# Seasandwpy/viso

Measured on AMD Instinct MI355X. Metric: stereo frames/sec at 1242x375 grey, 1/2/4/8 GPUs; pose RMSE vs reference, higher is better.
Workload: dtype f64

## Files before the change

### include/viso/viso.hpp

```cpp
#ifndef VISO_HPP
#define VISO_HPP

#include <algorithm>
#include <array>
#include <cmath>
#include <cstdint>
#include <functional>
#include <memory>
#include <stdexcept>
#include <string>
#include <mutex>
#include <vector>

#include "viso_c.h"

namespace viso {

inline void check(int rc, const char* what) {
    if (rc != VISO_OK) throw std::runtime_error(std::string(what) + " failed: " + std::to_string(rc));
}

using Pose = std::array<double, 12>;
using V3d = std::array<double, 3>;
using V2d = std::array<double, 2>;
// ... 202 lines not shown
        const Viso* v_;
        mutable std::vector<Pose> cache_;
    };
    PoseLog poses{this};

    std::vector<V3d> GetPoints() const {
        size_t n = 0;
        check(viso_get_points(ctx_, nullptr, 0, &n), "viso_get_points");
        std::vector<V3d> out(n);
        if (n) check(viso_get_points(ctx_, out.front().data(), n, &n), "viso_get_points");
        return out;
    }

    size_t num_poses() const {
        size_t n = 0;
        check(viso_get_poses(ctx_, nullptr, 0, &n), "viso_get_poses");
        return n;
    }

    std::vector<Pose> fetch_poses() const {
        size_t n = 0;
        check(viso_get_poses(ctx_, nullptr, 0, &n), "viso_get_poses");
        std::vector<Pose> out(n);
        if (n) check(viso_get_poses(ctx_, out.front().data(), n, &n), "viso_get_poses");
        return out;
    }

    int state() const {
        int32_t s = 0;
        check(viso_get_state(ctx_, &s), "viso_get_state");
        return s;
    }

    void SetMonoKeyframes(int interval, int ngood_permille = 500, int cell = 16, double min_parallax_deg = 0.25) {
        check(viso_set_mono_keyframes(ctx_, interval, ngood_permille, cell, min_parallax_deg),
              "viso_set_mono_keyframes");
    }
    void SetBundleAdjust(int iterations) { check(viso_set_bundle_adjust(ctx_, iterations), "viso_set_bundle_adjust"); }

    void SetMapWindow(int window, int cell = 16) { check(viso_set_map_window(ctx_, window, cell), "viso_set_map_window"); }
    std::array<int64_t, 8> MapWindow() const {
        std::array<int64_t, 8> info{};
        check(viso_get_map_window(ctx_, info.data()), "viso_get_map_window");
        return info;
    }
    std::vector<int32_t> GetPointHosts() const {
        size_t n = 0;
        check(viso_get_point_hosts(ctx_, nullptr, 0, &n), "viso_get_point_hosts");
        std::vector<int32_t> out(n);
        if (n) check(viso_get_point_hosts(ctx_, out.data(), n, &n), "viso_get_point_hosts");
        return out;
    }

    void SetPoseRefine(int iterations, double huber_px = 1.0, double max_shift_px = 8.0) {
        check(viso_set_pose_refine(ctx_, iterations, huber_px, max_shift_px), "viso_set_pose_refine");
    }
    std::array<double, 8> PoseRefine() const {
        std::array<double, 8> report{};
        check(viso_get_pose_refine(ctx_, report.data()), "viso_get_pose_refine");
        return report;
    }

    void SetPointCull(int interval, int max_fail_run = 3, double reproj_px = 2.0, int min_points = 50) {
        check(viso_set_point_cull(ctx_, interval, max_fail_run, reproj_px, min_points), "viso_set_point_cull");
    }
    std::array<int64_t, 8> PointCull() const {
// ... 109 lines not shown
```

### include/viso/viso_c.h

```cpp
#ifndef VISO_C_H
#define VISO_C_H

#include <stddef.h>
#include <stdint.h>

#ifdef __cplusplus
extern "C" {
#endif

#define VISO_OK 0
#define VISO_ERR_ARG (-1)
#define VISO_ERR_HIP (-2)
#define VISO_ERR_CAPACITY (-3)
#define VISO_ERR_STATE (-4)
#define VISO_ERR_NODEVICE (-5)

#define VISO_STATE_INITIALIZATION 0
#define VISO_STATE_RUNNING 1
#define VISO_STATE_FINISHED 2

typedef struct viso_params {
    double fx, fy, cx, cy;
    int32_t width, height;
    int32_t reinitialize_after;
// ... 54 lines not shown
#define VISO_KERNEL_RANSAC 3
#define VISO_KERNEL_SELECT 4
#define VISO_KERNEL_DIRECT 5
#define VISO_KERNEL_LKALIGN 6
#define VISO_KERNEL_STEREO 7
#define VISO_KERNEL_UPLOAD 8
#define VISO_KERNEL_MAPWIN 9
#define VISO_KERNEL_REFINE 10
#define VISO_KERNEL_CULL 11
#define VISO_KERNEL_POINTS 12
#define VISO_KERNEL_LKWARP 13
#define VISO_KERNEL_SEEDS 14
#define VISO_KERNEL_COUNT 15
int viso_timing_enable(viso_ctx* ctx, int32_t enable);
int viso_timing_select(viso_ctx* ctx, uint32_t kernel_mask);
int viso_timing_get(viso_ctx* ctx, int32_t kernel, int64_t* launches, double* total_ms);


int viso_pyramid_dims(int32_t width, int32_t height, int32_t dims[8], size_t* total_bytes);

int viso_pyramid(viso_ctx* ctx, const uint8_t* images, int32_t n, int32_t width, int32_t height,
                 uint8_t* out);

int viso_fast(viso_ctx* ctx, const uint8_t* image, int32_t width, int32_t height, int32_t thresh,
              int32_t* xs, int32_t* ys, int32_t* scores, size_t cap, size_t* n);

int viso_klt(viso_ctx* ctx, const uint8_t* ref_pyr, const uint8_t* cur_pyr, int32_t width,
             int32_t height, const float* kp1, float* kp2, uint8_t* success, int32_t n);

int viso_direct_pose(viso_ctx* ctx, const uint8_t* last_pyr, const uint8_t* cur_pyr,
                     int32_t width, int32_t height, const double* points, int32_t n_points,
                     const double pose_last[12], double pose_io[12]);

int viso_lk_align(viso_ctx* ctx, const uint8_t* kf_pyrs, const double* kf_poses, int32_t n_kf,
                  const uint8_t* cur_pyr, const double cur_pose[12], int32_t width,
                  int32_t height, const double* points, int32_t n_points, int32_t* pair_kf,
                  uint8_t* success, double* uv_before, double* uv_after);

int viso_pose_2d2d(viso_ctx* ctx, const double* p1, const double* p2, int32_t n, double R[9],
                   double T[3], uint8_t* inliers, double* points3d, double* candidates,
                   double stats[8]);

int viso_stereo_match(viso_ctx* ctx, const uint8_t* left, const uint8_t* right, int32_t width,
                      int32_t height, const int32_t* xs, const int32_t* ys, int32_t n,
                      int32_t max_disp, int32_t* disparity, int32_t* sad);

int viso_set_stereo(viso_ctx* ctx, double baseline, int32_t max_disp, int32_t min_disp);

int viso_set_keyframes(viso_ctx* ctx, int32_t interval, int32_t ngood_permille);

int viso_set_mono_keyframes(viso_ctx* ctx, int32_t interval, int32_t ngood_permille, int32_t cell,
                            double min_parallax_deg);
int viso_mono_points(viso_ctx* ctx, const uint8_t* cur_pyr, const uint8_t* kf_pyr, int32_t width,
                     int32_t height, const double pose_c[12], const double pose_k[12],
                     const double* points, int32_t n_points, int32_t cell, double min_parallax_deg,
                     double* new_points, int32_t* winners_xy, uint8_t* accept, size_t cap, size_t* n,
                     int32_t counts[4]);

int viso_set_map_window(viso_ctx* ctx, int32_t window, int32_t cell);
int viso_get_map_window(viso_ctx* ctx, int64_t info[8]);
int viso_get_point_hosts(viso_ctx* ctx, int32_t* host, size_t cap, size_t* n);
int viso_map_retire(viso_ctx* ctx, int32_t width, int32_t height, const double pose_c[12],
                    const double* kf_poses, int32_t n_kf, const double* points, const int32_t* host,
                    int32_t n, int32_t cell, double* out_points, int32_t* out_host, uint8_t* keep,
                    size_t* n_out, int32_t counts[4]);

// ... 72 lines not shown
```

### viso_amd/_lib.py

```python
from __future__ import annotations

import ctypes
import os

_HERE = os.path.dirname(os.path.abspath(__file__))
LIB_PATH = os.environ.get("VISO_LIB") or os.path.join(_HERE, "libviso_amd.so")

VISO_OK = 0
ERRORS = {-1: "VISO_ERR_ARG", -2: "VISO_ERR_HIP", -3: "VISO_ERR_CAPACITY",
          -4: "VISO_ERR_STATE", -5: "VISO_ERR_NODEVICE"}

STATE_INITIALIZATION, STATE_RUNNING, STATE_FINISHED = 0, 1, 2
KERNEL_IDS = {"pyramid": 0, "fast": 1, "klt": 2, "ransac": 3, "select": 4, "direct": 5,
              "lkalign": 6, "stereo": 7, "upload": 8, "mapwin": 9, "refine": 10, "cull": 11,
              "points": 12, "lkwarp": 13, "seeds": 14}


class VisoError(RuntimeError):
    def __init__(self, fn: str, rc: int):
        super().__init__(f"{fn} failed: {ERRORS.get(rc, rc)}")
        self.rc = rc


class viso_params(ctypes.Structure):
# ... 13 lines not shown
    ]


_vp = ctypes.c_void_p
_i32 = ctypes.c_int32
_sz = ctypes.c_size_t
_d = ctypes.c_double

SIGNATURES = {
    "viso_default_params": [_vp, _d, _d, _d, _d, _i32, _i32],
    "viso_create": [_vp, ctypes.c_int, _vp],
    "viso_destroy": [_vp],
    "viso_process_frame": [_vp, _vp, _i32, _i32, _i32],
    "viso_process_stereo": [_vp, _vp, _vp, _vp],
    "viso_process_frames_device": [_vp, _vp, _vp, _i32, _sz],
    "viso_synchronize": [_vp],
    "viso_get_state": [_vp, _vp],
    "viso_get_poses": [_vp, _vp, _sz, _vp],
    "viso_get_points": [_vp, _vp, _sz, _vp],
    "viso_get_init_tracks": [_vp, _vp, _vp, _vp, _sz, _vp],
    "viso_get_alignment": [_vp, _vp, _vp, _vp, _vp, _sz, _vp],
    "viso_get_frame_stats": [_vp, _vp],
    "viso_set_frame_log": [_vp, _i32],
    "viso_get_config": [_vp, _vp],
    "viso_get_frame_log": [_vp, _vp, _sz, _vp],
    "viso_timing_enable": [_vp, _i32],
    "viso_timing_select": [_vp, ctypes.c_uint32],
    "viso_timing_get": [_vp, _i32, _vp, _vp],
    "viso_pyramid_dims": [_i32, _i32, _vp, _vp],
    "viso_pyramid": [_vp, _vp, _i32, _i32, _i32, _vp],
    "viso_fast": [_vp, _vp, _i32, _i32, _i32, _vp, _vp, _vp, _sz, _vp],
    "viso_klt": [_vp, _vp, _vp, _i32, _i32, _vp, _vp, _vp, _i32],
    "viso_direct_pose": [_vp, _vp, _vp, _i32, _i32, _vp, _i32, _vp, _vp],
    "viso_lk_align": [_vp, _vp, _vp, _i32, _vp, _vp, _i32, _i32, _vp, _i32, _vp, _vp, _vp,
                      _vp],
    "viso_pose_2d2d": [_vp, _vp, _vp, _i32, _vp, _vp, _vp, _vp, _vp, _vp],
    "viso_stereo_match": [_vp, _vp, _vp, _i32, _i32, _vp, _vp, _i32, _i32, _vp, _vp],
    "viso_set_stereo": [_vp, _d, _i32, _i32],
    "viso_set_keyframes": [_vp, _i32, _i32],
    "viso_set_bundle_adjust": [_vp, _i32],
    "viso_get_keyframe_poses": [_vp, _vp, _sz, _vp],
    "viso_set_mono_keyframes": [_vp, _i32, _i32, _i32, _d],
    "viso_mono_points": [_vp, _vp, _vp, _i32, _i32, _vp, _vp, _vp, _i32, _i32, _d, _vp, _vp, _vp, _sz, _vp,
                         _vp],
    "viso_photometric_ba": [_vp, _vp, _i32, _vp, _vp, _vp, _i32, _i32, _vp],
    "viso_set_map_window": [_vp, _i32, _i32],
    "viso_get_map_window": [_vp, _vp],
    "viso_get_point_hosts": [_vp, _vp, _sz, _vp],
    "viso_map_retire": [_vp, _i32, _i32, _vp, _vp, _i32, _vp, _vp, _i32, _i32, _vp, _vp, _vp, _vp, _vp],
    "viso_set_pose_refine": [_vp, _i32, _d, _d],
    "viso_get_pose_refine": [_vp, _vp],
    "viso_refine_pose": [_vp, _vp, _vp, _vp, _vp, _vp, _i32, _vp, _i32, _d, _d, _vp, _vp],
    "viso_set_point_cull": [_vp, _i32, _i32, _d, _i32],
    "viso_get_point_cull": [_vp, _vp],
    "viso_get_point_tracks": [_vp, _vp, _sz, _vp],
    "viso_point_tracks_update": [_vp, _vp, _vp, _vp, _vp, _i32, _vp, _d, _vp, _vp],
    "viso_points_cull": [_vp, _vp, _vp, _vp, _i32, _i32, _i32, _vp, _vp, _vp, _vp, _vp, _vp],
    "viso_set_point_refine": [_vp, _i32, _i32, _i32, _d, _d, _i32, _d],
    "viso_get_point_refine": [_vp, _vp],
    "viso_get_point_refine_status": [_vp, _vp, _vp, _sz, _vp],
    "viso_point_obs_record": [_vp, _vp, _vp, _vp, _vp, _i32, _d, _vp, _vp],
    "viso_points_refine": [_vp, _vp, _vp, _i32, _vp, _i32, _vp, _i32, _vp, _vp, _i32, _d, _i32, _d, _vp, _vp, _vp,
                           _vp, _vp],
    "viso_set_lk_warp": [_vp, _i32, _d],
    "viso_get_lk_warp": [_vp, _vp],
    "viso_get_lk_warp_rows": [_vp, _vp, _vp, _vp, _sz, _vp],
# ... 98 lines not shown
```

### viso_amd/api.py

```python
from __future__ import annotations

import ctypes

import numpy as np

from . import _lib

_ctx_cache: dict = {}


def _p(a: np.ndarray | None):
    return None if a is None else a.ctypes.data


def pyramid_dims(width: int, height: int):
    dims = np.zeros(8, np.int32)
    total = ctypes.c_size_t(0)
    _lib.call("viso_pyramid_dims", width, height, _p(dims), ctypes.byref(total))
    return [(int(dims[2 * l]), int(dims[2 * l + 1])) for l in range(4)], int(total.value)


def default_params(fx=517.3, fy=516.5, cx=325.1, cy=249.7, width=640, height=480, **kw):
    p = _lib.viso_params()
    _lib.call("viso_default_params", ctypes.byref(p), fx, fy, cx, cy, width, height)
# ... 40 lines not shown
        _lib.call("viso_pyramid", self.h, _p(images), n, w, h, _p(out))
        return out

    def fast(self, image: np.ndarray, thresh: int = 50, cap: int = 1 << 20):
        image = np.ascontiguousarray(image, dtype=np.uint8)
        h, w = image.shape
        xs = np.zeros(cap, np.int32)
        ys = np.zeros(cap, np.int32)
        sc = np.zeros(cap, np.int32)
        n = ctypes.c_size_t(0)
        _lib.call("viso_fast", self.h, _p(image), w, h, thresh, _p(xs), _p(ys), _p(sc), cap,
                  ctypes.byref(n))
        m = min(n.value, cap)
        return xs[:m].copy(), ys[:m].copy(), sc[:m].copy()

    def klt(self, ref_pyr: np.ndarray, cur_pyr: np.ndarray, width: int, height: int,
            kp1: np.ndarray, kp2: np.ndarray):
        kp1 = np.ascontiguousarray(kp1, dtype=np.float32)
        kp2 = np.ascontiguousarray(kp2, dtype=np.float32).copy()
        n = kp1.shape[0]
        succ = np.zeros(n, np.uint8)
        _lib.call("viso_klt", self.h, _p(np.ascontiguousarray(ref_pyr)),
                  _p(np.ascontiguousarray(cur_pyr)), width, height, _p(kp1), _p(kp2), _p(succ), n)
        return kp2, succ

    def direct_pose(self, last_pyr, cur_pyr, width, height, points, pose_last, pose_init):
        pts = np.ascontiguousarray(points, dtype=np.float64).reshape(-1, 3)
        pl = np.ascontiguousarray(pose_last, dtype=np.float64).reshape(12)
        pio = np.ascontiguousarray(pose_init, dtype=np.float64).reshape(12).copy()
        _lib.call("viso_direct_pose", self.h, _p(np.ascontiguousarray(last_pyr)),
                  _p(np.ascontiguousarray(cur_pyr)), width, height, _p(pts), pts.shape[0],
                  _p(pl), _p(pio))
        return pio

    def lk_align(self, kf_pyrs, kf_poses, cur_pyr, cur_pose, width, height, points):
        kfp = np.ascontiguousarray(np.stack(kf_pyrs) if isinstance(kf_pyrs, (list, tuple))
                                   else kf_pyrs, dtype=np.uint8)
        kposes = np.ascontiguousarray(kf_poses, dtype=np.float64).reshape(-1, 12)
        pts = np.ascontiguousarray(points, dtype=np.float64).reshape(-1, 3)
        n = pts.shape[0]
        pk = np.zeros(n, np.int32)
        sc = np.zeros(n, np.uint8)
        ub = np.zeros((n, 2), np.float64)
        ua = np.zeros((n, 2), np.float64)
        cp = np.ascontiguousarray(cur_pose, dtype=np.float64).reshape(12)
        _lib.call("viso_lk_align", self.h, _p(kfp), _p(kposes), kposes.shape[0],
                  _p(np.ascontiguousarray(cur_pyr)), _p(cp), width, height, _p(pts), n, _p(pk),
                  _p(sc), _p(ub), _p(ua))
        return pk, sc, ub, ua

    def lk_align_warped(self, kf_pyrs, kf_poses, cur_pyr, cur_pose, width, height, points,
                        max_area_ratio: float = 64.0):
        kfp = np.ascontiguousarray(np.stack(kf_pyrs) if isinstance(kf_pyrs, (list, tuple))
                                   else kf_pyrs, dtype=np.uint8)
        kposes = np.ascontiguousarray(kf_poses, dtype=np.float64).reshape(-1, 12)
        pts = np.ascontiguousarray(points, dtype=np.float64).reshape(-1, 3)
        n = pts.shape[0]
        pk = np.zeros(n, np.int32)
        sc = np.zeros(n, np.uint8)
        ub = np.zeros((n, 2), np.float64)
        ua = np.zeros((n, 2), np.float64)
        A = np.zeros((n, 4), np.float64)
        sh = np.zeros(n, np.int8)
        st = np.zeros(n, np.uint8)
        cp = np.ascontiguousarray(cur_pose, dtype=np.float64).reshape(12)
        _lib.call("viso_lk_align_warped", self.h, _p(kfp), _p(kposes), kposes.shape[0],
# ... 297 lines not shown
```

### viso_amd/csrc/context.hip

```cpp
#include <algorithm>
#include <cstdio>
#include <cstring>
#include <new>
#include <vector>

#include "context.hpp"

using namespace viso;

namespace viso {

int DevBuf::ensure(size_t need) {
    if (need <= bytes) return VISO_OK;
    if (ptr) {
        VISO_HIP_CHECK(hipFree(ptr));
        ptr = nullptr;
        bytes = 0;
    }
    size_t b = std::max<size_t>(need, 256);
    VISO_HIP_CHECK(hipMalloc(&ptr, b));
    bytes = b;
    return VISO_OK;
}

// ... 265 lines not shown
        return VISO_ERR_ARG;
    if (int rc = c->settle()) return rc;
    if (n > 0 && !points) return VISO_ERR_ARG;
    VISO_HIP_CHECK(hipSetDevice(c->device));
    PyrGeom g = make_geom(width, height);
    Bump b;
    size_t o_l = b.take(g.bytes), o_c = b.take(g.bytes), o_p = b.take(24 * (size_t)std::max(n, 1)),
           o_pl = b.take(96), o_pio = b.take(96), o_ds = b.take(direct_scratch_bytes());
    int rc = c->scratch_a.ensure(b.off);
    if (rc) return rc;
    char* base = (char*)c->scratch_a.ptr;
    VISO_HIP_CHECK(hipMemcpyAsync(base + o_l, last_pyr, g.bytes, hipMemcpyHostToDevice, c->stream));
    VISO_HIP_CHECK(hipMemcpyAsync(base + o_c, cur_pyr, g.bytes, hipMemcpyHostToDevice, c->stream));
    if (n > 0)
        VISO_HIP_CHECK(hipMemcpyAsync(base + o_p, points, 24 * (size_t)n, hipMemcpyHostToDevice, c->stream));
    VISO_HIP_CHECK(hipMemcpyAsync(base + o_pl, pose_last, 96, hipMemcpyHostToDevice, c->stream));
    VISO_HIP_CHECK(hipMemcpyAsync(base + o_pio, pose_io, 96, hipMemcpyHostToDevice, c->stream));
    const double K[4] = {c->p.fx, c->p.fy, c->p.cx, c->p.cy};
    {
        TimedRegion t(c->timing, VISO_KERNEL_DIRECT, c->stream);
        launch_direct_pose(frame_from_base((const uint8_t*)(base + o_l), g),
                           frame_from_base((const uint8_t*)(base + o_c), g), g, K,
                           (const double*)(base + o_p), n, (const double*)(base + o_pl),
                           (const double*)(base + o_pio), direct_scratch_at(base + o_ds), nullptr,
                           (double*)(base + o_pio), nullptr, -1, c->stream, c->p.precision,
                           c->direct_scalar_pass);
    }
    VISO_HIP_CHECK(hipGetLastError());
    VISO_HIP_CHECK(hipMemcpyAsync(pose_io, base + o_pio, 96, hipMemcpyDeviceToHost, c->stream));
    VISO_HIP_CHECK(hipStreamSynchronize(c->stream));
    return VISO_OK;
}

static int lk_align_stage(viso_ctx* c, const uint8_t* kf_pyrs, const double* kf_poses, int32_t n_kf,
                          const uint8_t* cur_pyr, const double cur_pose[12], int32_t width, int32_t height,
                          const double* points, int32_t n, int32_t* pair_kf, uint8_t* success,
                          double* uv_before, double* uv_after, bool warp, double max_area_ratio, double* A4,
                          int8_t* shift, uint8_t* status) {
    if (!c || !kf_pyrs || !kf_poses || n_kf <= 0 || n_kf > kMaxKeyframes || !cur_pyr || !cur_pose ||
        n < 0)
        return VISO_ERR_ARG;
    if (warp && !(max_area_ratio >= 4.0 && max_area_ratio <= 64.0)) return VISO_ERR_ARG;
    if (int rc = c->settle()) return rc;
    if (n == 0) return VISO_OK;
    if (!points || !pair_kf || !success || !uv_before || !uv_after) return VISO_ERR_ARG;
    if (warp && (!A4 || !shift || !status)) return VISO_ERR_ARG;
    VISO_HIP_CHECK(hipSetDevice(c->device));
    PyrGeom g = make_geom(width, height);
    Bump b;
    size_t o_kf = b.take(g.bytes * (size_t)n_kf), o_kp = b.take(96 * (size_t)n_kf),
           o_c = b.take(g.bytes), o_cp = b.take(96), o_p = b.take(24 * (size_t)n),
           o_pk = b.take(4 * (size_t)n), o_s = b.take((size_t)n), o_ub = b.take(16 * (size_t)n),
           o_ua = b.take(16 * (size_t)n);
    const size_t o_wa = warp ? b.take(32 * (size_t)n) : 0, o_ws = warp ? b.take((size_t)n) : 0,
                 o_wt = warp ? b.take((size_t)n) : 0;
    int rc = c->scratch_a.ensure(b.off);
    if (rc) return rc;
    char* base = (char*)c->scratch_a.ptr;
    VISO_HIP_CHECK(hipMemcpyAsync(base + o_kf, kf_pyrs, g.bytes * (size_t)n_kf, hipMemcpyHostToDevice, c->stream));
    VISO_HIP_CHECK(hipMemcpyAsync(base + o_kp, kf_poses, 96 * (size_t)n_kf, hipMemcpyHostToDevice, c->stream));
    VISO_HIP_CHECK(hipMemcpyAsync(base + o_c, cur_pyr, g.bytes, hipMemcpyHostToDevice, c->stream));
    VISO_HIP_CHECK(hipMemcpyAsync(base + o_cp, cur_pose, 96, hipMemcpyHostToDevice, c->stream));
    VISO_HIP_CHECK(hipMemcpyAsync(base + o_p, points, 24 * (size_t)n, hipMemcpyHostToDevice, c->stream));
    LkAlignArgs a{};
    for (int j = 0; j < n_kf; ++j) a.kf[j] = frame_from_base((const uint8_t*)(base + o_kf + g.bytes * j), g);
    a.kf_poses = (const double*)(base + o_kp);
// ... 177 lines not shown
```

### viso_amd/csrc/direct.hip

```cpp
#include <algorithm>
#include <cstring>

#include "device_math.hpp"
#include "direct_solve.hpp"
#include "kernels.hpp"

#ifdef VISO_PROBE
constexpr int kPRing = 4096;
constexpr int kPSt = 24;
__device__ unsigned long long g_plog[kPRing][kPSt];
__device__ unsigned long long g_pexit[kPRing];
constexpr int kPRingB = 512;
__device__ unsigned long long g_pblk[kPRingB][256][4];
__device__ unsigned long long g_pwave[kPRingB][256][16];
#ifdef VISO_PROBE_PT
constexpr int kPtRing = 128, kPtBlocks = 32, kPtStamps = 5;
__device__ unsigned long long g_ppt[kPtRing][kPtBlocks][16][kPtStamps];
#define PPT(k)                                                                                       \
    do {                                                                                             \
        if (blockIdx.x < kPtBlocks && (threadIdx.x & 63) == 0)                                       \
            g_ppt[a.probe_seq & (kPtRing - 1)][blockIdx.x][threadIdx.x >> 6][(k)] =                  \
                __builtin_amdgcn_s_memrealtime();                                                    \
    } while (0)
#endif
// ... 796 lines not shown
    const int k = act ? lane - kSpLanes * p : kSpLanes - 1;
    const int j = kSpPerHelper * helper + p;
    const bool valid = act && j < T && first + j < a.n;
    const double scale = kScale[lv];
    const int w = a.g.w[lv], h = a.g.h[lv];
    const double P[3] = {pf.P[j][0], pf.P[j][1], pf.P[j][2]};
    const double q = quotient_select(a.K, cur_pose, P, scale, k);
    const double Q0 = bperm_f64(q, kSpLanes * p), Q1 = bperm_f64(q, kSpLanes * p + 1);
    const double uc = scale * (Q0 * a.K.fx + a.K.cx);
    const double vc = scale * (Q1 * a.K.fy + a.K.cy);
    const double hp = 4.0;
    const bool in = inside_px(uc - hp, vc - hp, w, h) && inside_px(uc + hp, vc + hp, w, h);
    const int fu = (int)floor(uc), fv = (int)floor(vc);
    const bool whole = patch_in_window(pf.cw[j][2] != 0, pf.cw[j][0], pf.cw[j][1], fu, fv);
    const int cls = !in ? kClsOut : !whole ? kClsSample : patch_one_binade(uc, vc) ? kClsShared : kClsStraddle;
    const double xx = uc - floor(uc), yy = vc - floor(vc);
    const double w00 = (1 - xx) * (1 - yy), w10 = xx * (1 - yy), w01 = (1 - xx) * yy, w11 = xx * yy;
    const bool shared = cls == kClsShared;
    if (valid) {
        sp.v[j][k] = q;
        if (k == 0) {
            double2* v2 = reinterpret_cast<double2*>(&sp.v[j][12]);
            v2[0] = make_double2(shared ? w00 : uc, shared ? w10 : vc);
            v2[1] = make_double2(w01, w11);
            *reinterpret_cast<int4*>(sp.cls[j]) = make_int4(cls, fu, fv, 0);
        }
    }
    __builtin_amdgcn_fence(__ATOMIC_RELEASE, "workgroup");
    if (valid && k == 0) __hip_atomic_store(&sp.ready[j], 1, __ATOMIC_RELAXED, __HIP_MEMORY_SCOPE_WORKGROUP);
}

constexpr unsigned kSrcHere = 0xffffffffu;

template <bool FAST, bool LV16 = false, int W = kWaves>
__device__ void direct_tile_pf(const DirectArgs& a, const LevelPair& fp, int lv, const double* cur_pose, int b,
                               const PfLds& pf, bool merged, double* part, int* good, double* s_pts,
                               int* s_good, int* s_cnt = nullptr, double* s_qt = nullptr,
                               unsigned src_in = kSrcHere, SpLds* sp = nullptr) {
    const int wave = wave_id(), lane = threadIdx.x & 63;
    int first, T;
    tile_range(a, b, &first, &T);
    int good_cnt = 0;
    const unsigned src_lanes = FAST ? 0u : src_in != kSrcHere ? src_in : factored_sources();
    const bool sp_on = !FAST && W == kWaves && sp && s_cnt && T > kSpPoints - kSpHelpers && T <= kSpPoints;
    if (sp_on && wave >= kSpPoints) {
        __builtin_amdgcn_s_setprio(3);
        scalar_pass(a, lv, cur_pose, pf, first, T, wave - kSpPoints, *sp);
        __builtin_amdgcn_s_setprio(1);
    }
    for (int local = wave; local < T; local += W) {
        const int i = first + local;
        double f = 0.0;
        int idx = -1;
        bool ok = false;
        if (i < a.n) {
            RefSample r;
            if (merged) {
                merged_ref(a, fp, lv, pf, local, r);
                if (!FAST) ref_finish(r);
            } else if (!FAST) {
                pf_ref(pf, local, r);
            } else {
                r.P[0] = pf.P[local][0];
                r.P[1] = pf.P[local][1];
                r.P[2] = pf.P[local][2];
                r.ur = pf.ur[local];
                r.vr = pf.vr[local];
// ... 26 lines not shown
        }
        if (!ok) {
            if (lane < kSums) s_pts[local * kSums + lane] = 0.0;
        } else if ((!FAST || lane < 32) && idx >= 0) {
            s_pts[local * kSums + idx] = f;
        }
        good_cnt += ok ? 1 : 0;
    }
    if (lane == 0 && good_cnt) atomicAdd(s_good, good_cnt);
#ifdef VISO_PROBE
    if (threadIdx.x == 0 && blockIdx.x < 256) g_pblk[a.probe_seq & (kPRingB - 1)][blockIdx.x][2] = __builtin_amdgcn_s_memrealtime();
    if (lane == 0 && blockIdx.x < 256 && wave < 15)
        g_pwave[a.probe_seq & (kPRingB - 1)][blockIdx.x][wave] = __builtin_amdgcn_s_memrealtime();
#endif
    if (s_cnt && T <= 16) {
        const int nw = T < W ? T : W;
        if (wave >= nw) return;
        int prev = 0;
        if (lane == 0)
            prev = __hip_atomic_fetch_add(s_cnt, 1, __ATOMIC_ACQ_REL, __HIP_MEMORY_SCOPE_WORKGROUP);
        prev = __builtin_amdgcn_readfirstlane(prev);
        if (prev != nw - 1) return;
        __builtin_amdgcn_fence(__ATOMIC_ACQUIRE, "workgroup");
        if (lane < kSums) {
            double v[16];
#pragma unroll
            for (int j = 0; j < 16; ++j) v[j] = j < T ? s_pts[j * kSums + lane] : 0.0;
#pragma unroll
            for (int st = 1; st < 16; st <<= 1)
#pragma unroll
                for (int j = 0; j < 16; j += 2 * st) v[j] = v[j] + v[j + st];
            double r = v[0] + 0.0;
            r = r + 0.0;
            part[(size_t)lane * kMaxTiles + b] = r;
        }
        if (lane == 0) good[b] = __hip_atomic_load(s_good, __ATOMIC_RELAXED, __HIP_MEMORY_SCOPE_WORKGROUP);
#ifdef VISO_PROBE
        if (lane == 0 && blockIdx.x < 256)
            g_pwave[a.probe_seq & (kPRingB - 1)][blockIdx.x][15] = __builtin_amdgcn_s_memrealtime();
#endif
        return;
    }
    __syncthreads();
    for (int k = wave; k < kSums; k += W) {
        const double v = lane < T ? s_pts[lane * kSums + k] : 0.0;
        const double r = wave_tree_sum_dpp(v);
        if (lane == 0) part[(size_t)k * kMaxTiles + b] = r;
    }
    if (threadIdx.x == 0) good[b] = *s_good;
    __syncthreads();
}

__device__ inline void state_to_pose(const double* st, double* pose) {
    double q[4] = {st[0], st[1], st[2], st[3]};
    quat_to_matrix(q, pose);
    pose[9] = st[4];
    pose[10] = st[5];
    pose[11] = st[6];
}


__device__ inline void load_partials(const double* __restrict__ part, const int* __restrict__ good,
                                     int n_tiles, double* v, int& gg) {
    const int t = threadIdx.x;
    if (t < n_tiles) {
#pragma unroll
        for (int k = 0; k < kSums; ++k) v[k] = part[(size_t)k * kMaxTiles + t];
        gg = good[t];
    } else {
#pragma unroll
        for (int k = 0; k < kSums; ++k) v[k] = 0.0;
        gg = 0;
    }
}

__device__ inline void load_partials_paired(const double* __restrict__ part, const int* __restrict__ good,
                                            int n_tiles, double* a, int& gg) {
    const int t = threadIdx.x;
    const int t0 = (t & ~63) + 2 * (t & 31);
    if (t0 < n_tiles) {
        const bool has1 = t0 + 1 < n_tiles;
        const double2* __restrict__ p2 =
            reinterpret_cast<const double2*>(part + ((t & 32) ? (size_t)(kSums / 2) * kMaxTiles : 0) + t0);
#pragma unroll
        for (int k = 0; k < kSums / 2; ++k) {
            const double2 x = p2[(size_t)k * (kMaxTiles / 2)];
            a[k] = x.x + (has1 ? x.y : 0.0);
        }
    } else {
#pragma unroll
        for (int k = 0; k < kSums / 2; ++k) a[k] = 0.0;
    }
    gg = t < n_tiles ? good[t] : 0;
}

__device__ inline void reduce_partials(const double* v, int gg, SolveLds& L) {
    const int t = threadIdx.x, wave = t >> 6, lane = t & 63;
    if (t < 256) {
        int idx;
        const double f = reduce_scatter_28(v, &idx);
        if (lane < 32 && idx >= 0) L.red[wave][idx] = f;
        const int g = wave_sum_int(gg);
        if (lane == 0) L.g[wave] = g;
    }
    __syncthreads();
    if (t < kSums) L.S[t] = (L.red[0][t] + L.red[1][t]) + (L.red[2][t] + L.red[3][t]);
    if (t == 0) L.ngood = (L.g[0] + L.g[1]) + (L.g[2] + L.g[3]);
    __syncthreads();
}

__device__ inline void lds_barrier() { asm volatile("s_waitcnt lgkmcnt(0)\n\ts_barrier" ::: "memory"); }

template <bool FAST>
__device__ void solve_continue(const DirectArgs& a, const FramePair& fpair, int lv, SolveLds& L,
                               double* stats, double* s_pose, double* s_pts, int* s_good, PfLds& pf) {
    const int t = threadIdx.x, wave = t >> 6;
    double* part = a.s.cont_part + (size_t)blockIdx.x * kMaxTiles * kSums;
    int* good = a.s.cont_good + (size_t)blockIdx.x * kMaxTiles;
    const LevelPair fp = level_pair(fpair, lv);
// ... 210 lines not shown
            after_solve(a, merged, L, s_last, s_pose);
            s_good = 0;
        }
        __syncthreads();
        if (tiles) {
            double pose[12];
#pragma unroll
            for (int k = 0; k < 12; ++k) pose[k] = s_pose[k];
            prefetch_tile(a, lv, blockIdx.x, pose, merged ? s_last : a.fp.pose_last, true, wave, kWaves, s_pf);
        }
        __syncthreads();
    }
    if (wave == 0) PST(8);
#ifdef VISO_PROBE
    if (t == 0 && blockIdx.x < 256) g_pblk[a.probe_seq & (kPRingB - 1)][blockIdx.x][1] = __builtin_amdgcn_s_memrealtime();
#endif
    const int out = lv >= 0 ? lv : kLevels;
    if (blockIdx.x == 0 && t == 0 && !merged) {
        for (int k = 0; k < 7; ++k) a.s.state[out * kStateStride + k] = L.state[k];
        if (lv < 0 && a.pose_out) {
            store_frame_pose(a.pose_out, s_pose, a.ready);
            log_pose(a.log, a.log_host, a.log_index, s_pose);
            log_frame(a.flog, a.log_index, L);
        }
    }
    if (blockIdx.x == 0 && t == 0 && merged)
        for (int k = 0; k < 7; ++k) a.s.state[lv * kStateStride + k] = L.state[k];
    if (tiles) {
        LevelPair fp = level_pair(a.fp, lv);
        if (merged) fp.pose_last = s_last;
        double pose[12];
#pragma unroll
        for (int k = 0; k < 12; ++k) pose[k] = s_pose[k];
        direct_tile_pf<FAST>(a, fp, lv, pose, blockIdx.x, s_pf, merged, a.s.part + (size_t)lv * kMaxTiles * kSums,
                       a.s.good + lv * kMaxTiles, s_pts, &s_good, &s_cnt, qt, src_lanes,
                       SP ? &s_sp : nullptr);
    }
#ifdef VISO_PROBE
    __syncthreads();
    const unsigned long long t_exit = __builtin_amdgcn_s_memrealtime();
    const int slot = a.probe_seq & (kPRing - 1);
    if (t == 0 && blockIdx.x < 256) g_pblk[a.probe_seq & (kPRingB - 1)][blockIdx.x][3] = t_exit;
    if (blockIdx.x == 0 && t == 0) {
        pst[11] = t_exit;
        pst[15] = (unsigned long long)(lv + 1) | ((unsigned long long)merged << 8) |
                  ((unsigned long long)a.n_tiles << 16);
        for (int k = 0; k < kPSt; ++k) g_plog[slot][k] = pst[k];
    }
#endif
}

constexpr int kRigTiles = kMaxTiles;

__device__ __host__ inline int rig_reduce_waves(int n_tiles) { return n_tiles <= 64 ? 1 : n_tiles <= 128 ? 2 : 4; }

struct RigCamArgs {
    DirectArgs d;
    const double* Ad;
    double E[12];
};

struct RigArgs {
    RigCamArgs cam[kMaxRigCams];
    int n_cams;
    int tile_off[kMaxRigCams + 1];
    int level;
    double* state;
    const double* seed;
    double* stats;
// ... 320 lines not shown
__global__ void set_pose_kernel(double* dst, Pose12v p) {
    if (threadIdx.x < 12) dst[threadIdx.x] = p.v[threadIdx.x];
}

__global__ void map_create_kernel(double* __restrict__ cur_pose, Pose12v p, const double* __restrict__ pts_src,
                                  double* __restrict__ pts_dst, int n_dbl, const double* __restrict__ ref_pose,
                                  double* __restrict__ kf_poses) {
    const int t = blockIdx.x * blockDim.x + threadIdx.x;
    for (int i = t; i < n_dbl; i += gridDim.x * blockDim.x) pts_dst[i] = pts_src[i];
    if (blockIdx.x == 0 && threadIdx.x < 12) {
        cur_pose[threadIdx.x] = p.v[threadIdx.x];
        kf_poses[threadIdx.x] = ref_pose[threadIdx.x];
        kf_poses[12 + threadIdx.x] = p.v[threadIdx.x];
    }
}

}

void launch_map_create(double* cur_pose, const double pose[12], const double* pts_src, double* pts_dst, int n_pts,
                       const double* ref_pose, double* kf_poses, hipStream_t stream) {
    Pose12v p;
    for (int k = 0; k < 12; ++k) p.v[k] = pose[k];
    const int n_dbl = 3 * n_pts;
    const int blocks = std::max(1, std::min((n_dbl + 255) / 256, 64));
    map_create_kernel<<<blocks, 256, 0, stream>>>(cur_pose, p, pts_src, pts_dst, n_dbl, ref_pose, kf_poses);
}

void launch_set_pose(double* dst, const double src[12], hipStream_t stream) {
    Pose12v p;
    for (int k = 0; k < 12; ++k) p.v[k] = src[k];
    set_pose_kernel<<<1, 64, 0, stream>>>(dst, p);
}

size_t direct_scratch_bytes() {
    return (size_t)kLevels * kMaxTiles * kSums * 8 + (size_t)kLevels * kMaxTiles * 4 +
           (size_t)(kLevels + 1) * kStateStride * 8 + (size_t)kMaxTiles * kMaxTiles * kSums * 8 +
           (size_t)kMaxTiles * kMaxTiles * 4 + 5 * 256;
}

DirectScratch direct_scratch_at(void* base) {
    auto align = [](size_t o) { return (o + 255) & ~(size_t)255; };
    char* b = (char*)base;
    size_t o = 0;
    DirectScratch s;
    s.part = (double*)(b + o);
    o = align(o + (size_t)kLevels * kMaxTiles * kSums * 8);
    s.good = (int*)(b + o);
    o = align(o + (size_t)kLevels * kMaxTiles * 4);
    s.state = (double*)(b + o);
    o = align(o + (size_t)(kLevels + 1) * kStateStride * 8);
    s.cont_part = (double*)(b + o);
    o = align(o + (size_t)kMaxTiles * kMaxTiles * kSums * 8);
    s.cont_good = (int*)(b + o);
    return s;
}

namespace {
#ifdef VISO_PROBE
static unsigned g_probe_host_seq = 0;
int next_probe_seq() { return (int)(g_probe_host_seq++); }
#else
int next_probe_seq() { return 0; }
#endif

DirectArgs direct_args(const FrameDev& last_pyr, const FrameDev& cur_pyr, const PyrGeom& g,
                       const double K[4], const double* points, int n, const double* pose_last12,
// ... 297 lines not shown
```

### viso_amd/csrc/direct_solve.hpp

```cpp
#pragma once

#include "common.hpp"
#include "device_math.hpp"


namespace viso {

constexpr int kSolveSums = 28;
constexpr int kSolveStateStride = 8;

struct SolveLds {
    double red[4][kSolveSums];
    double S[kSolveSums];
    int g[4];
    int ngood;
    double state[kSolveStateStride], best[kSolveStateStride];
    double cost, last_cost;
    int cont;
};

#define SPROBE(k)                                                   \
    do {                                                            \
        if (stamps) stamps[(k)] = __builtin_amdgcn_s_memrealtime(); \
    } while (0)
// ... 70 lines not shown
            for (int k = 0; k < 6; ++k) stats[38 + k] = L.S[21 + k];
            for (int k = 0; k < 6; ++k) stats[44 + k] = update[k];
        }
    }
    if (lane == 0) {
        int cont = 1;
        if (nan_update) {
            for (int k = 0; k < 7; ++k) L.state[k] = L.best[k];
            cont = 0;
        } else {
            for (int k = 0; k < 4; ++k) L.state[k] = T21.q[k];
            for (int k = 0; k < 3; ++k) L.state[4 + k] = T21.t[k];
            if (cost_up) {
                for (int k = 0; k < 7; ++k) L.state[k] = L.best[k];
                cont = 0;
            } else if (converged) {
                cont = 0;
            } else {
                for (int k = 0; k < 7; ++k) L.best[k] = L.state[k];
                L.last_cost = cost;
            }
        }
        L.cost = cost;
        L.cont = cont;
    }
}



__device__ __attribute__((always_inline)) inline void solve_after_lu(SolveLds& L, const double* A, const int* tr,
                                                                      double h, int iter, double* stats,
                                                                      unsigned long long* stamps);

template <bool QL = false>
__device__ __attribute__((always_inline)) inline void solve_wave0_rep(SolveLds& L, int iter, double* stats,
                                   unsigned long long* stamps = nullptr) {
    const int lane = threadIdx.x & 63;
    const int row = lane / 6, col = lane - 6 * (lane / 6);
    const bool in = lane < 36;
    const int r0 = row < col ? row : col, c0 = row < col ? col : row;
    const double h = in ? L.S[r0 * 6 - (r0 * (r0 - 1)) / 2 + (c0 - r0)] : 0.0;
    double A[36];
    int tr[6];
#ifdef VISO_LU_TWICE
#pragma clang loop unroll(disable)
    for (int rep = 0; rep < 2; ++rep) {
#endif
#pragma unroll
    for (int r = 0; r < 6; ++r)
#pragma unroll
        for (int c = 0; c < 6; ++c) {
            const int r1 = r < c ? r : c, c1 = r < c ? c : r;
            A[6 * r + c] = L.S[r1 * 6 - (r1 * (r1 - 1)) / 2 + (c1 - r1)];
        }
#pragma unroll
    for (int k = 0; k < 6; ++k) {
        int p = k;
        double best = fabs(A[7 * k]);
#pragma unroll
        for (int i = k + 1; i < 6; ++i) {
            const double s = fabs(A[6 * i + k]);
            if (s > best) {
                best = s;
                p = i;
            }
        }
        p = __builtin_amdgcn_readfirstlane(p);
        tr[k] = p;
        if (__builtin_amdgcn_readfirstlane(best != 0.0 ? 1 : 0)) {
#pragma unroll
            for (int i = k + 1; i < 6; ++i) {
                if (p == i) {
#pragma unroll
                    for (int c = 0; c < 6; ++c) {
                        const double tmp = A[6 * k + c];
                        A[6 * k + c] = A[6 * i + c];
                        A[6 * i + c] = tmp;
                    }
                }
            }
            const double piv = A[7 * k];
            if (QL && k < 4) {
                double num = A[6 * (k + 1) + k];
#pragma unroll
                for (int i = k + 2; i < 6; ++i) num = (lane == i - k - 1) ? A[6 * i + k] : num;
                const double q = num / piv;
#pragma unroll
                for (int i = k + 1; i < 6; ++i) A[6 * i + k] = readlane_f64(q, i - k - 1);
            } else {
#pragma unroll
                for (int i = k + 1; i < 6; ++i) A[6 * i + k] = A[6 * i + k] / piv;
            }
        }
#pragma unroll
        for (int i = k + 1; i < 6; ++i)
#pragma unroll
            for (int c = k + 1; c < 6; ++c) A[6 * i + c] = A[6 * i + c] - A[6 * i + k] * A[6 * k + c];
    }
#ifdef VISO_LU_TWICE
    if (rep == 0) {
        asm volatile("" ::"v"(A[35]), "v"(A[0]));
        if (stamps) stamps[4] = __builtin_amdgcn_s_memrealtime();
    }
    }
#endif
    SPROBE(0);
    solve_after_lu(L, A, tr, h, iter, stats, stamps);
}

__device__ __attribute__((always_inline)) inline void solve_after_lu(SolveLds& L, const double* A, const int* tr,
                                                                      double h, int iter, double* stats,
                                                                      unsigned long long* stamps) {
// ... 174 lines not shown
```

### viso_amd/csrc/kernels.hpp

```cpp
#pragma once

#include "../../include/viso/viso_c.h"
#include "common.hpp"

namespace viso {

void launch_pyramid(const PyrGeom& g, uint8_t* base, int n_images, size_t img_stride,
                    hipStream_t stream);
constexpr int kPyrBatch = 128;
struct FastScratch {
    int* cnt = nullptr;
    int* tot = nullptr;
    int* lst = nullptr;
};

struct FastPre {
    const uint8_t* img = nullptr;
    int w = 0, h = 0, thresh = 0;
    FastScratch s;
    bool done = false;
};

struct PyrOwn {
    int img;
// ... 259 lines not shown
    int n_kf;
    const double* poses;
    const uint8_t* valid;
    const double* uv;
    size_t stride;
    int m;
    int iterations, min_obs;
    double huber, max_rel_sigma;
    uint8_t* status;
    uint8_t* steps;
    double* costs;
    int* counts;
    unsigned long long* moved_total;
};
void launch_point_obs(const PointObsArgs& a, hipStream_t stream);
void launch_point_refine(const PointRefineArgs& a, hipStream_t stream);

constexpr int kMaxMapPoints = 16384;
struct DirectScratch {
    double* part = nullptr;
    int* good = nullptr;
    double* state = nullptr;
    double* cont_part = nullptr;
    int* cont_good = nullptr;
};
size_t direct_scratch_bytes();
DirectScratch direct_scratch_at(void* base);
void launch_direct_pose(const FrameDev& last, const FrameDev& cur, const PyrGeom& g,
                        const double K[4], const double* points, int n,
                        const double* pose_last12, const double* pose_seed12,
                        const DirectScratch& s, double* stats, double* pose_out, double* log,
                        int log_index, hipStream_t stream, int precision = VISO_PRECISION_FAITHFUL,
                        bool scalar_pass = true);
struct DirectPrev {
    FrameDev last, cur;
    const double* pose_last12;
    double* pose_out;
    double* log;
    int log_index;
    int* ready = nullptr;
    double* log_host = nullptr;
    double* flog = nullptr;
};
bool direct_fits_background();
void launch_direct_levels(const FrameDev& last, const FrameDev& cur, const PyrGeom& g,
                          const double K[4], const double* points, int n,
                          const double* pose_last12, const double* pose_seed12,
                          const DirectScratch& s, double* stats, const DirectPrev* merge,
                          hipStream_t stream, int precision = VISO_PRECISION_FAITHFUL, bool bg = false,
                          bool scalar_pass = true);
void launch_direct_final(const FrameDev& last, const FrameDev& cur, const PyrGeom& g,
                         const double K[4], const double* points, int n,
                         const double* pose_last12, const DirectScratch& s, double* stats,
                         double* pose_out, double* log, int log_index, hipStream_t stream,
                         int precision = VISO_PRECISION_FAITHFUL, int* ready = nullptr,
                         double* log_host = nullptr, double* flog = nullptr);
constexpr int kMaxRigCams = 4;
struct RigCamDev {
    FrameDev last, cur;
    const double* points;
    int n;
    const double* pose_last12;
    double E[12];
    const double* Ad;
    void* scratch;
};
// ... 15 lines not shown
```

Measured before the change: 21670.

## Interleave direct-pose partial sums and hand-code LU row exchange

Direct-pose tile partial sums are now written in a paired, interleaved layout, so the reducer reads each lane's pair as one contiguous double2 stride instead of computing split-half offsets. The 6x6 LU pivot row swap is rewritten as inline assembly that branches on the scalar pivot index instead of using unrolled predicated swaps. The lower-triangle loads go through an opaque pointer, likely to stop the compiler merging them. A new viso_direct_solve API with a standalone solve kernel is also added, exposing the solver for testing.

After: 22210 (median of 6 runs). 1.02x the previous value.

```diff
diff --git a/include/viso/viso.hpp b/include/viso/viso.hpp
--- a/include/viso/viso.hpp
+++ b/include/viso/viso.hpp
@@ -258,6 +258,15 @@
         return s;
     }
 
+    std::pair<std::array<double, 50>, std::array<double, 7>> DirectSolve(const std::array<double, 28>& sums,
+                                                                         int n_good,
+                                                                         const std::array<double, 7>& state) const {
+        std::pair<std::array<double, 50>, std::array<double, 7>> out{};
+        check(viso_direct_solve(ctx_, sums.data(), n_good, state.data(), out.first.data(), out.second.data()),
+              "viso_direct_solve");
+        return out;
+    }
+
     void SetMonoKeyframes(int interval, int ngood_permille = 500, int cell = 16, double min_parallax_deg = 0.25) {
         check(viso_set_mono_keyframes(ctx_, interval, ngood_permille, cell, min_parallax_deg),
               "viso_set_mono_keyframes");
diff --git a/include/viso/viso_c.h b/include/viso/viso_c.h
--- a/include/viso/viso_c.h
+++ b/include/viso/viso_c.h
@@ -110,6 +110,9 @@
                      int32_t width, int32_t height, const double* points, int32_t n_points,
                      const double pose_last[12], double pose_io[12]);
 
+int viso_direct_solve(viso_ctx* ctx, const double sums[28], int32_t n_good, const double state[7],
+                      double stats[50], double state_out[7]);
+
 int viso_lk_align(viso_ctx* ctx, const uint8_t* kf_pyrs, const double* kf_poses, int32_t n_kf,
                   const uint8_t* cur_pyr, const double cur_pose[12], int32_t width,
                   int32_t height, const double* points, int32_t n_points, int32_t* pair_kf,
diff --git a/viso_amd/_lib.py b/viso_amd/_lib.py
--- a/viso_amd/_lib.py
+++ b/viso_amd/_lib.py
@@ -69,6 +69,7 @@
     "viso_fast": [_vp, _vp, _i32, _i32, _i32, _vp, _vp, _vp, _sz, _vp],
     "viso_klt": [_vp, _vp, _vp, _i32, _i32, _vp, _vp, _vp, _i32],
     "viso_direct_pose": [_vp, _vp, _vp, _i32, _i32, _vp, _i32, _vp, _vp],
+    "viso_direct_solve": [_vp, _vp, _i32, _vp, _vp, _vp],
     "viso_lk_align": [_vp, _vp, _vp, _i32, _vp, _vp, _i32, _i32, _vp, _i32, _vp, _vp, _vp,
                       _vp],
     "viso_pose_2d2d": [_vp, _vp, _vp, _i32, _vp, _vp, _vp, _vp, _vp, _vp],
diff --git a/viso_amd/api.py b/viso_amd/api.py
--- a/viso_amd/api.py
+++ b/viso_amd/api.py
@@ -96,6 +96,14 @@
                   _p(np.ascontiguousarray(cur_pyr)), width, height, _p(pts), pts.shape[0],
                   _p(pl), _p(pio))
         return pio
+
+    def direct_solve(self, sums, n_good, state):
+        s = np.ascontiguousarray(sums, dtype=np.float64).reshape(28)
+        st = np.ascontiguousarray(state, dtype=np.float64).reshape(7)
+        stats = np.zeros(50, np.float64)
+        out = np.zeros(7, np.float64)
+        _lib.call("viso_direct_solve", self.h, _p(s), int(n_good), _p(st), _p(stats), _p(out))
+        return stats, out
 
     def lk_align(self, kf_pyrs, kf_poses, cur_pyr, cur_pose, width, height, points):
         kfp = np.ascontiguousarray(np.stack(kf_pyrs) if isinstance(kf_pyrs, (list, tuple))
diff --git a/viso_amd/csrc/context.hip b/viso_amd/csrc/context.hip
--- a/viso_amd/csrc/context.hip
+++ b/viso_amd/csrc/context.hip
@@ -321,6 +321,27 @@
     return VISO_OK;
 }
 
+int viso_direct_solve(viso_ctx* c, const double sums[28], int32_t n_good, const double state[7],
+                      double stats[50], double state_out[7]) {
+    if (!c || !sums || !state || !stats || !state_out) return VISO_ERR_ARG;
+    if (int rc = c->settle()) return rc;
+    VISO_HIP_CHECK(hipSetDevice(c->device));
+    Bump b;
+    size_t o_s = b.take(28 * 8), o_st = b.take(7 * 8), o_out = b.take(50 * 8), o_so = b.take(7 * 8);
+    int rc = c->scratch_a.ensure(b.off);
+    if (rc) return rc;
+    char* base = (char*)c->scratch_a.ptr;
+    VISO_HIP_CHECK(hipMemcpyAsync(base + o_s, sums, 28 * 8, hipMemcpyHostToDevice, c->stream));
+    VISO_HIP_CHECK(hipMemcpyAsync(base + o_st, state, 7 * 8, hipMemcpyHostToDevice, c->stream));
+    launch_direct_solve((const double*)(base + o_s), n_good, (const double*)(base + o_st), (double*)(base + o_out),
+                        (double*)(base + o_so), c->stream);
+    VISO_HIP_CHECK(hipGetLastError());
+    VISO_HIP_CHECK(hipMemcpyAsync(stats, base + o_out, 50 * 8, hipMemcpyDeviceToHost, c->stream));
+    VISO_HIP_CHECK(hipMemcpyAsync(state_out, base + o_so, 7 * 8, hipMemcpyDeviceToHost, c->stream));
+    VISO_HIP_CHECK(hipStreamSynchronize(c->stream));
+    return VISO_OK;
+}
+
 static int lk_align_stage(viso_ctx* c, const uint8_t* kf_pyrs, const double* kf_poses, int32_t n_kf,
                           const uint8_t* cur_pyr, const double cur_pose[12], int32_t width, int32_t height,
                           const double* points, int32_t n, int32_t* pair_kf, uint8_t* success,
diff --git a/viso_amd/csrc/direct.hip b/viso_amd/csrc/direct.hip
--- a/viso_amd/csrc/direct.hip
+++ b/viso_amd/csrc/direct.hip
@@ -852,7 +852,14 @@
 
 constexpr unsigned kSrcHere = 0xffffffffu;
 
-template <bool FAST, bool LV16 = false, int W = kWaves>
+template <bool PAIRED>
+__device__ inline size_t partial_index(int k, int b) {
+    if (!PAIRED) return (size_t)k * kMaxTiles + b;
+    const int h = k >= kSums / 2 ? 1 : 0;
+    return (size_t)((((k - h * (kSums / 2)) * 4 + (b >> 6)) * 2 + h) * 64 + (b & 63));
+}
+
+template <bool FAST, bool LV16 = false, int W = kWaves, bool PAIRED = false>
 __device__ void direct_tile_pf(const DirectArgs& a, const LevelPair& fp, int lv, const double* cur_pose, int b,
                                const PfLds& pf, bool merged, double* part, int* good, double* s_pts,
                                int* s_good, int* s_cnt = nullptr, double* s_qt = nullptr,
@@ -945,7 +952,7 @@
                 for (int j = 0; j < 16; j += 2 * st) v[j] = v[j] + v[j + st];
             double r = v[0] + 0.0;
             r = r + 0.0;
-            part[(size_t)lane * kMaxTiles + b] = r;
+            part[partial_index<PAIRED>(lane, b)] = r;
         }
         if (lane == 0) good[b] = __hip_atomic_load(s_good, __ATOMIC_RELAXED, __HIP_MEMORY_SCOPE_WORKGROUP);
 #ifdef VISO_PROBE
@@ -958,7 +965,7 @@
     for (int k = wave; k < kSums; k += W) {
         const double v = lane < T ? s_pts[lane * kSums + k] : 0.0;
         const double r = wave_tree_sum_dpp(v);
-        if (lane == 0) part[(size_t)k * kMaxTiles + b] = r;
+        if (lane == 0) part[partial_index<PAIRED>(k, b)] = r;
     }
     if (threadIdx.x == 0) good[b] = *s_good;
     __syncthreads();
@@ -993,11 +1000,10 @@
     const int t0 = (t & ~63) + 2 * (t & 31);
     if (t0 < n_tiles) {
         const bool has1 = t0 + 1 < n_tiles;
-        const double2* __restrict__ p2 =
-            reinterpret_cast<const double2*>(part + ((t & 32) ? (size_t)(kSums / 2) * kMaxTiles : 0) + t0);
+        const double2* __restrict__ p2 = reinterpret_cast<const double2*>(part) + t;
 #pragma unroll
         for (int k = 0; k < kSums / 2; ++k) {
-            const double2 x = p2[(size_t)k * (kMaxTiles / 2)];
+            const double2 x = p2[(size_t)k * kMaxTiles];
             a[k] = x.x + (has1 ? x.y : 0.0);
         }
     } else {
@@ -1274,9 +1280,10 @@
         double pose[12];
 #pragma unroll
         for (int k = 0; k < 12; ++k) pose[k] = s_pose[k];
-        direct_tile_pf<FAST>(a, fp, lv, pose, blockIdx.x, s_pf, merged, a.s.part + (size_t)lv * kMaxTiles * kSums,
-                       a.s.good + lv * kMaxTiles, s_pts, &s_good, &s_cnt, qt, src_lanes,
-                       SP ? &s_sp : nullptr);
+        direct_tile_pf<FAST, false, kWaves, true>(a, fp, lv, pose, blockIdx.x, s_pf, merged,
+                                                  a.s.part + (size_t)lv * kMaxTiles * kSums,
+                                                  a.s.good + lv * kMaxTiles, s_pts, &s_good, &s_cnt, qt,
+                                                  src_lanes, SP ? &s_sp : nullptr);
     }
 #ifdef VISO_PROBE
     __syncthreads();
@@ -1663,6 +1670,33 @@
     set_pose_kernel<<<1, 64, 0, stream>>>(dst, p);
 }
 
+namespace {
+__global__ __launch_bounds__(64) void direct_solve_kernel(const double* __restrict__ sums, int ngood,
+                                                          const double* __restrict__ state_in,
+                                                          double* __restrict__ stats, double* __restrict__ state_out) {
+    __shared__ SolveLds L;
+    const int lane = threadIdx.x;
+    if (lane < kSolveSums) L.S[lane] = sums[lane];
+    if (lane == 0) {
+        for (int k = 0; k < 7; ++k) L.state[k] = L.best[k] = state_in[k];
+        L.ngood = ngood;
+        L.cost = 0.0;
+        L.last_cost = 0.0;
+        L.cont = 0;
+    }
+    __syncthreads();
+    solve_wave0(L, 0, stats);
+    __syncthreads();
+    if (lane < 7) state_out[lane] = L.state[lane];
+}
+}
+
+void launch_direct_solve(const double* sums28, int ngood, const double* state7, double* stats50, double* state_out7,
+                         hipStream_t stream) {
+    static_assert(kStats == 50, "viso_direct_solve's stats row");
+    direct_solve_kernel<<<1, 64, 0, stream>>>(sums28, ngood, state7, stats50, state_out7);
+}
+
 size_t direct_scratch_bytes() {
     return (size_t)kLevels * kMaxTiles * kSums * 8 + (size_t)kLevels * kMaxTiles * 4 +
            (size_t)(kLevels + 1) * kStateStride * 8 + (size_t)kMaxTiles * kMaxTiles * kSums * 8 +
diff --git a/viso_amd/csrc/direct_solve.hpp b/viso_amd/csrc/direct_solve.hpp
--- a/viso_amd/csrc/direct_solve.hpp
+++ b/viso_amd/csrc/direct_solve.hpp
@@ -126,6 +126,52 @@
                                                                       double h, int iter, double* stats,
                                                                       unsigned long long* stamps);
 
+#define VISO_LU_X1(r, c)                                                        \
+    "v_mov_b64 %[t], %[a" #c "]\n\tv_mov_b64 %[a" #c "], %[" #r #c "]\n\t" \
+    "v_mov_b64 %[" #r #c "], %[t]\n\t"
+#define VISO_LU_XROW(r) \
+    VISO_LU_X1(r, 0) VISO_LU_X1(r, 1) VISO_LU_X1(r, 2) VISO_LU_X1(r, 3) VISO_LU_X1(r, 4) VISO_LU_X1(r, 5)
+#define VISO_LU_SKIP(k) "s_cmp_eq_u32 %[p], " #k "\n\ts_cbranch_scc1 9f\n\t"
+#define VISO_LU_CASE(i, lbl, r) \
+    "s_cmp_lg_u32 %[p], " #i "\n\ts_cbranch_scc1 " #lbl "f\n\t" VISO_LU_XROW(r) "s_branch 9f\n" #lbl ":\n\t"
+#define VISO_LU_END "9:"
+#define VISO_LU_ROW(n, r)                                                                              \
+    [n##0] "+v"(A[6 * (r) + 0]), [n##1] "+v"(A[6 * (r) + 1]), [n##2] "+v"(A[6 * (r) + 2]), \
+        [n##3] "+v"(A[6 * (r) + 3]), [n##4] "+v"(A[6 * (r) + 4]), [n##5] "+v"(A[6 * (r) + 5])
+template <int K>
+__device__ __attribute__((always_inline)) inline void lu_exchange(double* A, int p) {
+    double t;
+    if constexpr (K == 0)
+        asm(VISO_LU_SKIP(0) VISO_LU_CASE(1, 1, b) VISO_LU_CASE(2, 2, c) VISO_LU_CASE(3, 3, d) VISO_LU_CASE(4, 4, e)
+                VISO_LU_XROW(f) VISO_LU_END
+            : VISO_LU_ROW(a, 0), VISO_LU_ROW(b, 1), VISO_LU_ROW(c, 2), VISO_LU_ROW(d, 3), VISO_LU_ROW(e, 4),
+              VISO_LU_ROW(f, 5), [t] "=&v"(t)
+            : [p] "s"(p)
+            : "scc");
+    else if constexpr (K == 1)
+        asm(VISO_LU_SKIP(1) VISO_LU_CASE(2, 1, b) VISO_LU_CASE(3, 2, c) VISO_LU_CASE(4, 3, d) VISO_LU_XROW(e)
+                VISO_LU_END
+            : VISO_LU_ROW(a, 1), VISO_LU_ROW(b, 2), VISO_LU_ROW(c, 3), VISO_LU_ROW(d, 4), VISO_LU_ROW(e, 5),
+              [t] "=&v"(t)
+            : [p] "s"(p)
+            : "scc");
+    else if constexpr (K == 2)
+        asm(VISO_LU_SKIP(2) VISO_LU_CASE(3, 1, b) VISO_LU_CASE(4, 2, c) VISO_LU_XROW(d) VISO_LU_END
+            : VISO_LU_ROW(a, 2), VISO_LU_ROW(b, 3), VISO_LU_ROW(c, 4), VISO_LU_ROW(d, 5), [t] "=&v"(t)
+            : [p] "s"(p)
+            : "scc");
+    else if constexpr (K == 3)
+        asm(VISO_LU_SKIP(3) VISO_LU_CASE(4, 1, b) VISO_LU_XROW(c) VISO_LU_END
+            : VISO_LU_ROW(a, 3), VISO_LU_ROW(b, 4), VISO_LU_ROW(c, 5), [t] "=&v"(t)
+            : [p] "s"(p)
+            : "scc");
+    else if constexpr (K == 4)
+        asm(VISO_LU_SKIP(4) VISO_LU_XROW(b) VISO_LU_END
+            : VISO_LU_ROW(a, 4), VISO_LU_ROW(b, 5), [t] "=&v"(t)
+            : [p] "s"(p)
+            : "scc");
+}
+
 template <bool QL = false>
 __device__ __attribute__((always_inline)) inline void solve_wave0_rep(SolveLds& L, int iter, double* stats,
                                    unsigned long long* stamps = nullptr) {
@@ -140,12 +186,15 @@
 #pragma clang loop unroll(disable)
     for (int rep = 0; rep < 2; ++rep) {
 #endif
+    int lower = 0;
+    asm("" : "+v"(lower));
+    const double* SL = L.S + lower;
 #pragma unroll
     for (int r = 0; r < 6; ++r)
 #pragma unroll
         for (int c = 0; c < 6; ++c) {
             const int r1 = r < c ? r : c, c1 = r < c ? c : r;
-            A[6 * r + c] = L.S[r1 * 6 - (r1 * (r1 - 1)) / 2 + (c1 - r1)];
+            A[6 * r + c] = (r > c ? SL : L.S)[r1 * 6 - (r1 * (r1 - 1)) / 2 + (c1 - r1)];
         }
 #pragma unroll
     for (int k = 0; k < 6; ++k) {
@@ -162,16 +211,13 @@
         p = __builtin_amdgcn_readfirstlane(p);
         tr[k] = p;
         if (__builtin_amdgcn_readfirstlane(best != 0.0 ? 1 : 0)) {
-#pragma unroll
-            for (int i = k + 1; i < 6; ++i) {
-                if (p == i) {
-#pragma unroll
-                    for (int c = 0; c < 6; ++c) {
-                        const double tmp = A[6 * k + c];
-                        A[6 * k + c] = A[6 * i + c];
-                        A[6 * i + c] = tmp;
-                    }
-                }
+            switch (k) {
+                case 0: lu_exchange<0>(A, p); break;
+                case 1: lu_exchange<1>(A, p); break;
+                case 2: lu_exchange<2>(A, p); break;
+                case 3: lu_exchange<3>(A, p); break;
+                case 4: lu_exchange<4>(A, p); break;
+                default: break;
             }
             const double piv = A[7 * k];
             if (QL && k < 4) {
diff --git a/viso_amd/csrc/kernels.hpp b/viso_amd/csrc/kernels.hpp
--- a/viso_amd/csrc/kernels.hpp
+++ b/viso_amd/csrc/kernels.hpp
@@ -315,6 +315,8 @@
                         const DirectScratch& s, double* stats, double* pose_out, double* log,
                         int log_index, hipStream_t stream, int precision = VISO_PRECISION_FAITHFUL,
                         bool scalar_pass = true);
+void launch_direct_solve(const double* sums28, int ngood, const double* state7, double* stats50,
+                         double* state_out7, hipStream_t stream);
 struct DirectPrev {
     FrameDev last, cur;
     const double* pose_last12;
```
